# dfm/emcee

Hardware: NVIDIA H100
Metric: walker-steps/sec (nwalkers x iters / s) (higher is better)
Workload: dtype f64

## Files before the change

emcee_b200/csrc/dense_dmma.cu:

```cuda
#include <math.h>

#include "draws.cuh"
#include "engine.cuh"
#include "tma.cuh"

namespace eb {

namespace {

constexpr int DMMA_CONSUMERS = 8;
constexpr int DMMA_THREADS = 64 * DMMA_CONSUMERS;
constexpr int NI = 2;
constexpr int DMMA_PRODUCER_REGS = 64;
constexpr int DMMA_CONSUMER_REGS = 192;
static_assert((DMMA_THREADS / 2) * (DMMA_PRODUCER_REGS + DMMA_CONSUMER_REGS) <= 65536, "register file of one SM");
__host__ __device__ constexpr bool dmma_rebalance(int KB, bool HAS_MEAN, bool BOUNDED) {
  return !BOUNDED && (KB >= 15 || (HAS_MEAN && KB >= 11));
}

__device__ __forceinline__ void dmma1688(double (&c)[4], double2 a01, double2 a23, double b0, double b1) {
  asm volatile(
      "mma.sync.aligned.m16n8k8.row.col.f64.f64.f64.f64 {%0,%1,%2,%3}, {%4,%5,%6,%7}, {%8,%9}, {%0,%1,%2,%3};"
      : "+d"(c[0]), "+d"(c[1]), "+d"(c[2]), "+d"(c[3])
      : "d"(a01.x), "d"(a01.y), "d"(a23.x), "d"(a23.y), "d"(b0), "d"(b1));
}

__host__ __device__ constexpr int col_pairs(int KB) { return (KB + 1) / 2; }
__host__ __device__ constexpr int factor_dmmas(int KB) { return col_pairs(KB) * (KB - col_pairs(KB) + 1); }
__host__ __device__ constexpr size_t factor_doubles(int KB) { return (size_t)factor_dmmas(KB) * 128; }
__host__ __device__ constexpr int row_stride(int KB) { return 8 * KB + 8; }

struct TileMeta {
  double factor[8];
  double log_u[8];
  double lp_old[8];
  int32_t w[8];
};

template <int KB>
struct SmemLayout {
  static constexpr size_t L_doubles = factor_doubles(KB);
  static constexpr size_t mu_doubles = 8 * KB;
  static constexpr size_t slot_doubles = 2 * 8 * row_stride(KB);
  static constexpr size_t off_mu = L_doubles;
  static constexpr size_t off_slots = off_mu + mu_doubles;
  static constexpr size_t off_meta = off_slots + DMMA_CONSUMERS * slot_doubles;
  static constexpr size_t meta_bytes = sizeof(TileMeta) * 2 * DMMA_CONSUMERS;
  static constexpr size_t off_bars_bytes = off_meta * sizeof(double) + meta_bytes;
  static constexpr int nbars = 1 + 3 * DMMA_CONSUMERS;
  static constexpr size_t off_abort_bytes = off_bars_bytes + nbars * sizeof(uint64_t);
  static constexpr size_t off_inbox_bytes = off_abort_bytes + 16;
  static constexpr size_t total_bytes = off_inbox_bytes + sizeof(int32_t) * 2 * 8 * DMMA_CONSUMERS;
};

template <int KB, bool HAS_MEAN>
__device__ __forceinline__ double tile_sumsq(const double (&q)[2 * KB], const double* sL, const double* sMu, int lane,
                                             int g, int t) {
  constexpr int NP = col_pairs(KB);
  double rs0 = 0.0, rs1 = 0.0;
  const double* aptr = sL + 2 * lane;
#pragma unroll
  for (int m0 = 0; m0 < NP; m0 += NI) {
    double c[NI][4];
#pragma unroll
    for (int n = 0; n < NI; ++n) c[n][0] = c[n][1] = c[n][2] = c[n][3] = 0.0;
#pragma unroll
    for (int j = 2 * m0; j < KB; ++j) {
      double x0 = q[2 * j + 0], x1 = q[2 * j + 1];
      if (HAS_MEAN) {
        const double2 m2 = *reinterpret_cast<const double2*>(sMu + 8 * j + 2 * t);
        x0 -= m2.x;
        x1 -= m2.y;
      }
#pragma unroll
      for (int n = 0; n < NI; ++n) {
        if (m0 + n < NP && j >= 2 * (m0 + n)) {
          const double2 a01 = *reinterpret_cast<const double2*>(aptr);
          const double2 a23 = *reinterpret_cast<const double2*>(aptr + 64);
          dmma1688(c[n], a01, a23, x0, x1);
          aptr += 128;
        }
      }
    }
#pragma unroll
    for (int n = 0; n < NI; ++n) {
      rs0 = fma(c[n][0], c[n][0], rs0);
      rs0 = fma(c[n][2], c[n][2], rs0);
      rs1 = fma(c[n][1], c[n][1], rs1);
      rs1 = fma(c[n][3], c[n][3], rs1);
    }
  }
#pragma unroll
  for (int o = 4; o < 32; o <<= 1) {
    rs0 += __shfl_xor_sync(0xffffffffu, rs0, o);
    rs1 += __shfl_xor_sync(0xffffffffu, rs1, o);
  }
  const double e = __shfl_sync(0xffffffffu, rs0, g >> 1), o = __shfl_sync(0xffffffffu, rs1, g >> 1);
  return (g & 1) ? o : e;
}

__device__ __forceinline__ bool grid_wait(const unsigned long long* counter, unsigned long long target, int* status) {
  const long long t0 = clock64();
  while (*reinterpret_cast<const volatile unsigned long long*>(counter) < target) {
    __nanosleep(32);
    if (clock64() - t0 > 60000000000ll) {
      atomicOr(status, FLAG_COMM_TIMEOUT);
      return false;
    }
  }
  __threadfence();
  return true;
}

__device__ __forceinline__ bool peer_wait(const unsigned* my_flags, int rank, int nranks, unsigned target, int lane,
                                          int* status) {
  bool ok = true;
  if (lane < nranks && lane != rank) {
    const volatile unsigned* f = my_flags + lane;
    const long long t0 = clock64();
    while ((int)(*f - target) < 0) {
      __nanosleep(64);
      if (clock64() - t0 > 60000000000ll) {
        atomicOr(status, FLAG_COMM_TIMEOUT);
        ok = false;
        break;
      }
    }
  }
  __threadfence_system();
  return __all_sync(0xffffffffu, ok);
}

template <int KB, bool HAS_MEAN, bool BOUNDED, bool TIMELINE>
__global__ void __launch_bounds__(DMMA_THREADS, 1)
    half_step_dense_dmma_kernel(const HalfStepArgs a, const HalfDesc d0, const HalfDesc* __restrict__ descs,
                                const int nhalf, unsigned long long* gbar, const unsigned long long gbar_base) {
  constexpr int D = 8 * KB;
  constexpr int RS = row_stride(KB);
  using SL = SmemLayout<KB>;
  extern __shared__ __align__(16) unsigned char smem_raw[];
  double* sL = reinterpret_cast<double*>(smem_raw);
  double* sMu = sL + SL::off_mu;
  double* sSlots = sL + SL::off_slots;
  TileMeta* sMeta = reinterpret_cast<TileMeta*>(sL + SL::off_meta);
  uint64_t* bars = reinterpret_cast<uint64_t*>(smem_raw + SL::off_bars_bytes);
  volatile int* sAbort = reinterpret_cast<volatile int*>(smem_raw + SL::off_abort_bytes);
  volatile int* sPeers = sAbort + 1;
  int32_t* sInbox = reinterpret_cast<int32_t*>(smem_raw + SL::off_inbox_bytes);
  uint64_t* barL = bars;
  uint64_t* barFull = bars + 1;
  uint64_t* barReady = bars + 1 + DMMA_CONSUMERS;
  uint64_t* barFree = bars + 1 + 2 * DMMA_CONSUMERS;

  const int tid = threadIdx.x, lane = tid & 31, warp = tid >> 5;
  const bool is_producer = warp >= DMMA_CONSUMERS;
  const int pair = is_producer ? warp - DMMA_CONSUMERS : warp;
  const int g = lane >> 2, t = lane & 3;

  if (tid == 0) {
    *sAbort = 0;
    *sPeers = 0;
    mbar_init(barL, 1);
    for (int c = 0; c < DMMA_CONSUMERS; ++c) {
      mbar_init(barFull + c, 1);
      mbar_init(barReady + c, 1);
      mbar_init(barFree + c, 1);
    }
    asm volatile("fence.mbarrier_init.release.cluster;" ::: "memory");
  }
  if (HAS_MEAN)
    for (int k = tid; k < D; k += DMMA_THREADS) sMu[k] = a.model.params[k];
  __syncthreads();
  const long long t_base = TIMELINE ? clock64() : 0;

  const int tstride = (int)gridDim.x * DMMA_CONSUMERS;
  const int tile0 = (int)blockIdx.x + (int)gridDim.x * pair;
  double* slot = sSlots + (size_t)pair * SL::slot_doubles;
  double* myS = slot + (size_t)g * RS + 2 * t;
  double* myC = myS + 8 * RS;
  TileMeta* meta = sMeta + 2 * pair;
  const bool multi = a.p2p_peer_flags != nullptr;
  unsigned k = 0;

  constexpr bool REBALANCE = dmma_rebalance(KB, HAS_MEAN, BOUNDED);
  if (is_producer) {
    if constexpr (REBALANCE) asm volatile("setmaxnreg.dec.sync.aligned.u32 %0;" ::"n"(DMMA_PRODUCER_REGS));
    long long* tlp = (TIMELINE && lane == 0)
                         ? a.timeline + ((size_t)blockIdx.x * DMMA_CONSUMERS + pair) * TL_TILES * TL_EVENTS : nullptr;
    const double dm1 = (double)a.D - 1.0;
    const int row = lane & 7;
    struct Prep {
      int32_t w, wp;
      double zz, factor, log_u, lp_old;
      bool valid, remote;
    };
    for (int h = 0; h < nhalf; ++h) {
      const HalfDesc d = (h == 0) ? d0 : descs[h];
      const int32_t* order = a.order + (size_t)d.order_step * a.N;
      const int2 rg = a.range ? a.range[(size_t)d.order_step * MAX_SPLITS + d.split] : make_int2(0, d.a_count);
      const int i_lo = rg.x, i_hi = rg.y;
      const int ntiles = (int)(((int64_t)i_hi - i_lo + 7) >> 3);
      const int64_t Nc = a.N - d.a_count;
      const int32_t* aperm = a.aperm ? a.aperm + (size_t)d.order_step * a.N + d.a_start : nullptr;
      auto prep = [&](int tile, bool with_lp) -> Prep {
        Prep p;
        int i = i_lo + tile * 8 + row;
        p.valid = i < i_hi;
        if (!p.valid) i = i_hi - 1;
        if (aperm) i = __ldg(aperm + i);
        const u32x4 A = prop_a(a.seed, d.step, (uint32_t)d.split, (uint32_t)i);
        p.zz = stretch_zz(A, a.p0);
        const int64_t r = stretch_rank(A, Nc);
        p.w = __ldg(order + d.a_start + i);
        p.wp = __ldg(order + complement_slot(r, d.a_start, d.a_count));
        p.log_u = log(accept_uniform(a.seed, d.step, (uint32_t)d.split, (uint32_t)i));
        p.factor = stretch_factor(dm1, p.zz);
        p.lp_old = with_lp ? a.logp[p.w] : 0.0;
        p.remote = multi && (p.wp / a.rows_per_rank != a.p2p_rank);
        return p;
      };
      auto peers_ready = [&]() -> bool {
        if (!multi || *sPeers > h) return true;
        if (pair == 0) {
          if (!peer_wait(a.p2p_my_flags, a.p2p_rank, a.p2p_nranks, a.p2p_wait + (unsigned)h, lane, a.status)) {
            *sAbort = 1;
            return false;
          }
          __syncwarp();
          if (lane == 0) *sPeers = h + 1;
        } else {
          while (*sPeers <= h) {
            if (*sAbort) return false;
            __nanosleep(64);
          }
        }
        asm volatile("fence.proxy.async;" ::: "memory");
        return true;
      };
      auto request = [&](const Prep& p, int lo, int hi) {
        if (lane >= lo && lane < hi) {
          const bool partner = lane >= 8;
          const int32_t wr = partner ? p.wp : p.w;
          const double* base =
              (partner && a.peer_coords != nullptr) ? a.peer_coords[wr / a.rows_per_rank] : a.coords;
          double* dst = slot + (size_t)(partner ? 8 : 0) * RS + (size_t)row * RS;
          if (partner)
            bulk_g2s(dst, base + (size_t)wr * D, (unsigned)(D * sizeof(double)), barFull + pair);
          else
            bulk_g2s_hint(dst, base + (size_t)wr * D, (unsigned)(D * sizeof(double)), barFull + pair,
                          l2_evict_first_policy());
        }
      };
      auto publish = [&](const Prep& p, int par) {
        TileMeta* m = meta + par;
        if (lane < 8) {
          m->factor[row] = p.factor;
          m->log_u[row] = p.log_u;
          m->lp_old[row] = p.lp_old;
          m->w[row] = p.valid ? p.w : -1;
        }
      };
      auto issue = [&](Prep& p, int par, bool load_lp) -> bool {
        if (__any_sync(0xffffffffu, p.remote) && !peers_ready()) return false;
        fence_async_smem();
        if (lane == 0) mbar_arrive_expect_tx(barFull + pair, 16u * D * (unsigned)sizeof(double));
        __syncwarp();
        request(p, 0, 16);
        if (load_lp) p.lp_old = a.logp[p.w];
        publish(p, par);
        return true;
      };
      Prep cur{}, nxt{};
      const bool early = h == 0 && a.dmma_early_own && tile0 < ntiles;
      if (early) {
        cur = prep(tile0, true);
        if (lane == 0) mbar_arrive_expect_tx(barFull + pair, 16u * D * (unsigned)sizeof(double));
        __syncwarp();
        if (tlp) tlp[6] = clock64() - t_base;
        request(cur, 0, 8);
      } else if (tile0 < ntiles) {
        cur = prep(tile0, false);
      }
      if (h == 0) {
        pdl_wait();
        pdl_launch_dependents();
        if (tlp) tlp[10] = clock64() - t_base;
        if (multi && !a.aperm && !peers_ready()) return;
        if (tile0 < ntiles) {
          if (a.dmma_stagger && pair >= DMMA_CONSUMERS / 2)
            mbar_wait_for(barFull + pair - DMMA_CONSUMERS / 2, 0, multi ? 40000 : 12000);
          if (tlp) {
            const long long t_req = clock64() - t_base;
            tlp[11] = t_req;
            if (!early) tlp[6] = t_req;
          }
          if (early) {
            request(cur, 8, 16);
            publish(cur, (int)(k & 1u));
          } else {
            if (!issue(cur, (int)(k & 1u), true)) return;
          }
        }
        if (pair == 0 && !peers_ready()) return;
        if (tile0 + tstride < ntiles) nxt = prep(tile0 + tstride, true);
      } else {
        if (tile0 + tstride < ntiles) nxt = prep(tile0 + tstride, false);
        bool ok = true;
        if (lane == 0) ok = grid_wait(gbar, gbar_base + (unsigned long long)h * gridDim.x, a.status);
        ok = __shfl_sync(0xffffffffu, ok, 0);
        if (!ok) {
          *sAbort = 1;
          return;
        }
        asm volatile("fence.proxy.async;" ::: "memory");
        if (tile0 < ntiles) {
          if (k > 0 && !mbar_wait_abortable(barFree + pair, (k - 1) & 1u, sAbort)) return;
          if (!issue(cur, (int)(k & 1u), true)) return;
        }
      }
      for (int tile = tile0; tile < ntiles; tile += tstride, ++k) {
        const double zz = __shfl_sync(0xffffffffu, cur.zz, g);
        if (!mbar_wait_abortable(barFull + pair, k & 1u, sAbort)) return;
        long long* tlq = (tlp && h == nhalf - 1 && (tile - tile0) / tstride < TL_TILES && lane == 0)
                             ? tlp + ((tile - tile0) / tstride) * TL_EVENTS : nullptr;
        if (tlq) tlq[7] = clock64() - t_base;
        if constexpr (BOUNDED) {
          bool in = true;
#pragma unroll
          for (int j = 0; j < KB; ++j) {
            const double2 s2 = *reinterpret_cast<const double2*>(myS + 8 * j);
            const double2 c2 = *reinterpret_cast<const double2*>(myC + 8 * j);
            const double2 q2 = make_double2(stretch_q(s2.x, c2.x, zz), stretch_q(s2.y, c2.y, zz));
            *reinterpret_cast<double2*>(myC + 8 * j) = q2;
            const double2 l2 = __ldg(reinterpret_cast<const double2*>(a.model.lo + 8 * j + 2 * t));
            const double2 h2 = __ldg(reinterpret_cast<const double2*>(a.model.hi + 8 * j + 2 * t));
            in &= (l2.x <= q2.x) & (q2.x <= h2.x) & (l2.y <= q2.y) & (q2.y <= h2.y);
          }
          in &= __shfl_xor_sync(0xffffffffu, in, 1);
          in &= __shfl_xor_sync(0xffffffffu, in, 2);
          if (t == 0) sInbox[(2 * pair + (k & 1u)) * 8 + g] = in ? 1 : 0;
        } else {
#pragma unroll
          for (int j = 0; j < KB; ++j) {
            const double2 s2 = *reinterpret_cast<const double2*>(myS + 8 * j);
            const double2 c2 = *reinterpret_cast<const double2*>(myC + 8 * j);
            *reinterpret_cast<double2*>(myC + 8 * j) =
                make_double2(stretch_q(s2.x, c2.x, zz), stretch_q(s2.y, c2.y, zz));
          }
        }
        __syncwarp();
        if (lane == 0) mbar_arrive(barReady + pair);
        if (tlq) tlq[8] = clock64() - t_base;
        if (tile + tstride < ntiles) {
          cur = nxt;
          if (!mbar_wait_abortable(barFree + pair, k & 1u, sAbort)) return;
          if (tlq && (tile - tile0) / tstride + 1 < TL_TILES)
            tlq[TL_EVENTS + 6] = clock64() - t_base;
          if (!issue(cur, (int)((k + 1) & 1u), h > 0 && tile == tile0)) return;
          if (tile + 2 * tstride < ntiles) nxt = prep(tile + 2 * tstride, true);
        }
      }
    }
    return;
  }

  if constexpr (REBALANCE) asm volatile("setmaxnreg.inc.sync.aligned.u32 %0;" ::"n"(DMMA_CONSUMER_REGS));
  if (tid == 0) {
    constexpr unsigned bytes = (unsigned)(SL::L_doubles * sizeof(double));
    mbar_arrive_expect_tx(barL, bytes);
    bulk_g2s(sL, a.model.chol, bytes, barL);
  }
  long long* tl = TIMELINE ? a.timeline + ((size_t)blockIdx.x * DMMA_CONSUMERS + pair) * TL_TILES * TL_EVENTS : nullptr;
  pdl_wait();
  pdl_launch_dependents();
  bool alive = mbar_wait_abortable_notrap(barL, 0, sAbort, a.status, FLAG_WAIT_TIMEOUT);
  if (TIMELINE && lane == 0) tl[9] = clock64() - t_base;
  for (int h = 0; h < nhalf; ++h) {
    const HalfDesc d = (h == 0) ? d0 : descs[h];
    const int2 rg = a.range ? a.range[(size_t)d.order_step * MAX_SPLITS + d.split] : make_int2(0, d.a_count);
    const int ntiles = (int)(((int64_t)rg.y - rg.x + 7) >> 3);
    unsigned kk = 0;
    bool peers_passed = false;
    for (int tile = tile0; alive && tile < ntiles; tile += tstride, ++k, ++kk) {
      const TileMeta* m = meta + (k & 1u);
      long long* tlk = (tl && h == nhalf - 1 && kk < TL_TILES && lane == 0) ? tl + kk * TL_EVENTS : nullptr;
      if (tlk) {
        tlk[0] = (long long)tile;
        tlk[1] = clock64() - t_base;
      }
      if (!mbar_wait_abortable_notrap(barReady + pair, k & 1u, sAbort, a.status, FLAG_WAIT_TIMEOUT)) {
        alive = false;
        break;
      }
      if (tlk) tlk[2] = clock64() - t_base;
      double q[2 * KB];
#pragma unroll
      for (int j = 0; j < KB; ++j) {
        const double2 q2 = *reinterpret_cast<const double2*>(myC + 8 * j);
        q[2 * j + 0] = q2.x;
        q[2 * j + 1] = q2.y;
      }
      __syncwarp();
      if (lane == 0) mbar_arrive(barFree + pair);
      if (tlk) tlk[3] = clock64() - t_base;

      const double rs = tile_sumsq<KB, HAS_MEAN>(q, sL, sMu, lane, g, t);
      const int32_t w = m->w[g];
      const double factor = m->factor[g], log_u = m->log_u[g], lp_old = m->lp_old[g];
      const double lp_new = (BOUNDED && sInbox[(2 * pair + (k & 1u)) * 8 + g] == 0) ? -INFINITY : -0.5 * rs;
      if (tlk) tlk[4] = clock64() - t_base;

      if (!isfinite(lp_new)) {
        bool any_inf = false, any_nan = false;
#pragma unroll
        for (int e = 0; e < 2 * KB; ++e) {
          any_inf |= isinf(q[e]);
          any_nan |= isnan(q[e]);
        }
        if (any_inf) atomicOr(a.status, FLAG_INF_PARAM);
        if (any_nan) atomicOr(a.status, FLAG_NAN_PARAM);
        if (isnan(lp_new)) atomicOr(a.status, FLAG_NAN_LOGPROB);
      }

      const double lnpdiff = lnpdiff_red_blue(factor, lp_new, lp_old);
      const bool acc = (w >= 0) && (lnpdiff > log_u);
      if (multi && !peers_passed) {
        while (*sPeers <= h) {
          if (*sAbort) break;
          __nanosleep(64);
        }
        peers_passed = !*sAbort;
        if (!peers_passed) {
          alive = false;
          break;
        }
      }
      if (acc) {
        double* dst = a.coords + (size_t)w * D + 2 * t;
#pragma unroll
        for (int j = 0; j < KB; ++j) *reinterpret_cast<double2*>(dst + 8 * j) = make_double2(q[2 * j], q[2 * j + 1]);
      }
      if (w >= 0 && t == 0) {
        if (acc) {
          a.logp[w] = lp_new;
          atomicAdd(a.nacc + w, 1ull);
        }
        a.accepted[w] = acc ? 1 : 0;
      }
      if (tlk) tlk[5] = clock64() - t_base;
    }
    if (h + 1 < nhalf) {
      __threadfence();
      asm volatile("bar.sync 1, %0;" ::"r"(32 * DMMA_CONSUMERS) : "memory");
      if (*sAbort) alive = false;
      if (tid == 0 && alive) {
        __threadfence();
        atomicAdd(gbar, 1ull);
      }
    }
  }
  if (multi) {
    __threadfence_system();
    asm volatile("bar.sync 1, %0;" ::"r"(32 * DMMA_CONSUMERS) : "memory");
    if (tid == 0 && !*sAbort) {
      const unsigned prev = atomicAdd(a.p2p_done, 1u);
      if (prev == gridDim.x - 1) {
        *a.p2p_done = 0;
        __threadfence_system();
        for (int r = 0; r < a.p2p_nranks; ++r)
          if (r != a.p2p_rank)
            atomicExch_system(a.p2p_peer_flags[r] + a.p2p_rank, a.p2p_signal + (unsigned)(nhalf - 1));
      }
    }
  }
}

template <int KB, bool HAS_MEAN>
__global__ void __launch_bounds__(256) logprob_dense_dmma_kernel(const ModelDev m, const double* __restrict__ x,
                                                                 const int64_t rows, double* __restrict__ out,
                                                                 int* status) {
  constexpr int D = 8 * KB;
  extern __shared__ __align__(16) unsigned char smem_raw[];
  double* sL = reinterpret_cast<double*>(smem_raw);
  double* sMu = sL + factor_doubles(KB);
  uint64_t* barL = reinterpret_cast<uint64_t*>(sMu + D);
  const int tid = threadIdx.x, lane = tid & 31, warp = tid >> 5;
  const int g = lane >> 2, t = lane & 3;
  if (tid == 0) {
    mbar_init(barL, 1);
    asm volatile("fence.mbarrier_init.release.cluster;" ::: "memory");
  }
  if (HAS_MEAN)
    for (int k = tid; k < D; k += blockDim.x) sMu[k] = m.params[k];
  __syncthreads();
  if (tid == 0) {
    constexpr unsigned bytes = (unsigned)(factor_doubles(KB) * sizeof(double));
    mbar_arrive_expect_tx(barL, bytes);
    bulk_g2s(sL, m.chol, bytes, barL);
  }
  const int64_t ntiles = (rows + 7) >> 3;
  bool waited = false;
  for (int64_t tile = (int64_t)blockIdx.x * 8 + warp; tile < ntiles; tile += (int64_t)gridDim.x * 8) {
    int64_t r = tile * 8 + g;
    const bool valid = r < rows;
    if (!valid) r = rows - 1;
    const double* src = x + (size_t)r * D + 2 * t;
    double q[2 * KB];
    bool any_inf = false, any_nan = false, in = true;
#pragma unroll
    for (int j = 0; j < KB; ++j) {
      const double2 v = __ldcg(reinterpret_cast<const double2*>(src + 8 * j));
      q[2 * j + 0] = v.x;
      q[2 * j + 1] = v.y;
      any_inf |= isinf(v.x) | isinf(v.y);
      any_nan |= isnan(v.x) | isnan(v.y);
      if (m.lo != nullptr) {
        const double2 l2 = __ldg(reinterpret_cast<const double2*>(m.lo + 8 * j + 2 * t));
        const double2 h2 = __ldg(reinterpret_cast<const double2*>(m.hi + 8 * j + 2 * t));
        in &= (l2.x <= v.x) & (v.x <= h2.x) & (l2.y <= v.y) & (v.y <= h2.y);
      }
    }
    in &= __shfl_xor_sync(0xffffffffu, in, 1);
    in &= __shfl_xor_sync(0xffffffffu, in, 2);
    if (valid && any_inf) atomicOr(status, FLAG_INF_PARAM);
    if (valid && any_nan) atomicOr(status, FLAG_NAN_PARAM);
    if (!waited) {
      mbar_wait(barL, 0);
      waited = true;
    }
    const double rs = tile_sumsq<KB, HAS_MEAN>(q, sL, sMu, lane, g, t);
    const double lp = in ? -0.5 * rs : -INFINITY;
    if (valid && t == 0) {
      out[r] = lp;
      if (isnan(lp)) atomicOr(status, FLAG_NAN_LOGPROB);
    }
  }
}

template <int KB>
cudaError_t launch_lp_t(const ModelDev& m, const double* x, int64_t rows, double* out, int* status, int sm_count,
                        cudaStream_t st) {
  const size_t smem = (factor_doubles(KB) + 8 * KB) * sizeof(double) + sizeof(uint64_t);
  const bool has_mean = m.s0 != 0.0;
  auto kern = has_mean ? logprob_dense_dmma_kernel<KB, true> : logprob_dense_dmma_kernel<KB, false>;
  if (smem > 48 * 1024) {
    cudaError_t e = cudaFuncSetAttribute(kern, cudaFuncAttributeMaxDynamicSharedMemorySize, (int)smem);
    if (e != cudaSuccess) return e;
  }
  if (rows <= 0) return cudaSuccess;
  const int64_t want = (((rows + 7) >> 3) + 7) / 8;
  const int grid = (int)(want < 2 * sm_count ? want : 2 * sm_count);
  kern<<<grid, 256, smem, st>>>(m, x, rows, out, status);
  return cudaGetLastError();
}

template <int KB>
cudaError_t launch_t(const HalfStepArgs& a, const HalfDesc& d0, const HalfDesc* descs_dev, int nhalf, int max_count,
                     unsigned long long* gbar, unsigned long long gbar_base, int sm_count, bool pdl, int* grid_out,
                     cudaStream_t st) {
  const size_t smem = SmemLayout<KB>::total_bytes;
  const bool has_mean = a.model.s0 != 0.0;
  const bool bounded = a.model.lo != nullptr;
  const bool timeline = a.timeline != nullptr;
  using Kern = decltype(&half_step_dense_dmma_kernel<KB, false, false, false>);
  static const Kern kerns[8] = {
      half_step_dense_dmma_kernel<KB, false, false, false>, half_step_dense_dmma_kernel<KB, true, false, false>,
      half_step_dense_dmma_kernel<KB, false, true, false>,  half_step_dense_dmma_kernel<KB, true, true, false>,
      half_step_dense_dmma_kernel<KB, false, false, true>,  half_step_dense_dmma_kernel<KB, true, false, true>,
      half_step_dense_dmma_kernel<KB, false, true, true>,   half_step_dense_dmma_kernel<KB, true, true, true>};
  const int variant = (has_mean ? 1 : 0) + (bounded ? 2 : 0) + (timeline ? 4 : 0);
  const Kern kern = kerns[variant];
  static bool configured[8][64] = {};
  int dev = 0;
  cudaGetDevice(&dev);
  if (dev < 0 || dev >= 64 || !configured[variant][dev]) {
    cudaError_t e = cudaFuncSetAttribute(kern, cudaFuncAttributeMaxDynamicSharedMemorySize, (int)smem);
    if (e != cudaSuccess) return e;
    if (dev >= 0 && dev < 64) configured[variant][dev] = true;
  }
  *grid_out = 0;
  if (max_count <= 0 || nhalf <= 0) return cudaSuccess;
  const int64_t ntiles = ((int64_t)max_count + 7) / 8;
  const int grid = (int)(ntiles < sm_count ? ntiles : sm_count);
  *grid_out = grid;
  HalfStepArgs args = a;
  HalfDesc first = d0;
  if (nhalf == 1) {
    cudaLaunchConfig_t cfg{};
    cfg.gridDim = dim3(grid);
    cfg.blockDim = dim3(DMMA_THREADS);
    cfg.dynamicSmemBytes = smem;
    cfg.stream = st;
    cudaLaunchAttribute attr[1];
    attr[0].id = cudaLaunchAttributeProgrammaticStreamSerialization;
    attr[0].val.programmaticStreamSerializationAllowed = 1;
    cfg.attrs = attr;
    cfg.numAttrs = pdl ? 1 : 0;
    return cudaLaunchKernelEx(&cfg, kern, args, first, descs_dev, nhalf, gbar, gbar_base);
  }
  void* params[] = {(void*)&args, (void*)&first, (void*)&descs_dev, (void*)&nhalf, (void*)&gbar, (void*)&gbar_base};
  return cudaLaunchCooperativeKernel((const void*)kern, dim3(grid), dim3(DMMA_THREADS), params, smem, st);
}

}

bool dense_dmma_supported(int D) { return D >= 8 && D <= 128 && D % 8 == 0; }

size_t dense_dmma_factor_doubles(int D) { return factor_doubles(D / 8); }

void dense_dmma_pack_factor(const double* L, int D, double* packed) {
  const int KB = D / 8, NP = col_pairs(KB);
  size_t idx = 0;
  for (int m0 = 0; m0 < NP; m0 += NI)
    for (int j = 2 * m0; j < KB; ++j)
      for (int n = 0; n < NI; ++n) {
        const int m = m0 + n;
        if (m >= NP || j < 2 * m) continue;
        for (int half = 0; half < 2; ++half)
          for (int lane = 0; lane < 32; ++lane) {
            const int g = lane >> 2, t = lane & 3, row = 8 * j + 2 * t + half;
            for (int hi = 0; hi < 2; ++hi) {
              const int col = 16 * m + 8 * hi + g;
              packed[idx++] = (col < D && col <= row) ? L[(size_t)row * D + col] : 0.0;
            }
          }
      }
}

cudaError_t launch_logprob_dense_dmma(const ModelDev& m, int D, const double* x, int64_t rows, double* out,
                                      int* status, int sm_count, cudaStream_t st) {
#define EB_LP_CASE(KB) \
  case 8 * KB:         \
    return launch_lp_t<KB>(m, x, rows, out, status, sm_count, st);
  switch (D) {
    EB_LP_CASE(1)
    EB_LP_CASE(2)
    EB_LP_CASE(3)
    EB_LP_CASE(4)
    EB_LP_CASE(5)
    EB_LP_CASE(6)
    EB_LP_CASE(7)
    EB_LP_CASE(8)
    EB_LP_CASE(9)
    EB_LP_CASE(10)
    EB_LP_CASE(11)
    EB_LP_CASE(12)
    EB_LP_CASE(13)
    EB_LP_CASE(14)
    EB_LP_CASE(15)
    EB_LP_CASE(16)
  }
#undef EB_LP_CASE
  return cudaErrorNotSupported;
}

cudaError_t launch_dense_dmma(const HalfStepArgs& a, const HalfDesc& d0, const HalfDesc* descs_dev, int nhalf,
                              int max_count, unsigned long long* gbar, unsigned long long gbar_base, int sm_count,
                              bool pdl, int* grid_out, cudaStream_t st) {
#define EB_DMMA_CASE(KB) \
  case 8 * KB:           \
    return launch_t<KB>(a, d0, descs_dev, nhalf, max_count, gbar, gbar_base, sm_count, pdl, grid_out, st);
  switch (a.D) {
    EB_DMMA_CASE(1)
    EB_DMMA_CASE(2)
    EB_DMMA_CASE(3)
    EB_DMMA_CASE(4)
    EB_DMMA_CASE(5)
    EB_DMMA_CASE(6)
    EB_DMMA_CASE(7)
    EB_DMMA_CASE(8)
    EB_DMMA_CASE(9)
    EB_DMMA_CASE(10)
    EB_DMMA_CASE(11)
    EB_DMMA_CASE(12)
    EB_DMMA_CASE(13)
    EB_DMMA_CASE(14)
    EB_DMMA_CASE(15)
    EB_DMMA_CASE(16)
  }
#undef EB_DMMA_CASE
  return cudaErrorNotSupported;
}

}
```

Before: 995.2 million.

## Move stretch-move computation from producer warp into consumers reading TMA data directly

The producer warp no longer waits for the bulk copy to land and then computes the stretched proposal back into shared memory. Consumers now wait on the TMA full barrier, compute q from the complementary and own coordinates with zz published in the tile metadata, and do the bounds check themselves. A separate per-parity ready barrier signals when the metadata is published. This removes a shared-memory round trip and a producer-consumer handoff from the critical path, at the cost of more consumer work and an extra barrier wait.

Result: no change. 988.1 million (median of 6 runs) (-0.7%).

```diff
diff --git a/emcee_b200/csrc/dense_dmma.cu b/emcee_b200/csrc/dense_dmma.cu
--- a/emcee_b200/csrc/dense_dmma.cu
+++ b/emcee_b200/csrc/dense_dmma.cu
@@ -31,6 +31,7 @@
 __host__ __device__ constexpr int row_stride(int KB) { return 8 * KB + 8; }
 
 struct TileMeta {
+  double zz[8];
   double factor[8];
   double log_u[8];
   double lp_old[8];
@@ -47,10 +48,9 @@
   static constexpr size_t off_meta = off_slots + DMMA_CONSUMERS * slot_doubles;
   static constexpr size_t meta_bytes = sizeof(TileMeta) * 2 * DMMA_CONSUMERS;
   static constexpr size_t off_bars_bytes = off_meta * sizeof(double) + meta_bytes;
-  static constexpr int nbars = 1 + 3 * DMMA_CONSUMERS;
+  static constexpr int nbars = 1 + 4 * DMMA_CONSUMERS;
   static constexpr size_t off_abort_bytes = off_bars_bytes + nbars * sizeof(uint64_t);
-  static constexpr size_t off_inbox_bytes = off_abort_bytes + 16;
-  static constexpr size_t total_bytes = off_inbox_bytes + sizeof(int32_t) * 2 * 8 * DMMA_CONSUMERS;
+  static constexpr size_t total_bytes = off_abort_bytes + 16;
 };
 
 template <int KB, bool HAS_MEAN>
@@ -146,11 +146,10 @@
   uint64_t* bars = reinterpret_cast<uint64_t*>(smem_raw + SL::off_bars_bytes);
   volatile int* sAbort = reinterpret_cast<volatile int*>(smem_raw + SL::off_abort_bytes);
   volatile int* sPeers = sAbort + 1;
-  int32_t* sInbox = reinterpret_cast<int32_t*>(smem_raw + SL::off_inbox_bytes);
   uint64_t* barL = bars;
   uint64_t* barFull = bars + 1;
-  uint64_t* barReady = bars + 1 + DMMA_CONSUMERS;
-  uint64_t* barFree = bars + 1 + 2 * DMMA_CONSUMERS;
+  uint64_t* barFree = bars + 1 + DMMA_CONSUMERS;
+  uint64_t* barReady = bars + 1 + 2 * DMMA_CONSUMERS;
 
   const int tid = threadIdx.x, lane = tid & 31, warp = tid >> 5;
   const bool is_producer = warp >= DMMA_CONSUMERS;
@@ -163,8 +162,9 @@
     mbar_init(barL, 1);
     for (int c = 0; c < DMMA_CONSUMERS; ++c) {
       mbar_init(barFull + c, 1);
-      mbar_init(barReady + c, 1);
       mbar_init(barFree + c, 1);
+      mbar_init(barReady + 2 * c, 1);
+      mbar_init(barReady + 2 * c + 1, 1);
     }
     asm volatile("fence.mbarrier_init.release.cluster;" ::: "memory");
   }
@@ -176,8 +176,8 @@
   const int tstride = (int)gridDim.x * DMMA_CONSUMERS;
   const int tile0 = (int)blockIdx.x + (int)gridDim.x * pair;
   double* slot = sSlots + (size_t)pair * SL::slot_doubles;
-  double* myS = slot + (size_t)g * RS + 2 * t;
-  double* myC = myS + 8 * RS;
+  const double* myS = slot + (size_t)g * RS + 2 * t;
+  const double* myC = myS + 8 * RS;
   TileMeta* meta = sMeta + 2 * pair;
   const bool multi = a.p2p_peer_flags != nullptr;
   unsigned k = 0;
@@ -187,6 +187,9 @@
     if constexpr (REBALANCE) asm volatile("setmaxnreg.dec.sync.aligned.u32 %0;" ::"n"(DMMA_PRODUCER_REGS));
     long long* tlp = (TIMELINE && lane == 0)
                          ? a.timeline + ((size_t)blockIdx.x * DMMA_CONSUMERS + pair) * TL_TILES * TL_EVENTS : nullptr;
+    auto stamp = [&](int i, int ev) {
+      if (tlp && i < TL_TILES) tlp[i * TL_EVENTS + ev] = clock64() - t_base;
+    };
     const double dm1 = (double)a.D - 1.0;
     const int row = lane & 7;
     struct Prep {
@@ -251,6 +254,12 @@
                           l2_evict_first_policy());
         }
       };
+      auto arm = [&](const Prep& p, int par) {
+        if (lane < 8) meta[par].zz[row] = p.zz;
+        __syncwarp();
+        if (lane == 0) mbar_arrive_expect_tx(barFull + pair, 16u * D * (unsigned)sizeof(double));
+        __syncwarp();
+      };
       auto publish = [&](const Prep& p, int par) {
         TileMeta* m = meta + par;
         if (lane < 8) {
@@ -259,12 +268,12 @@
           m->lp_old[row] = p.lp_old;
           m->w[row] = p.valid ? p.w : -1;
         }
+        __syncwarp();
+        if (lane == 0) mbar_arrive(barReady + 2 * pair + par);
       };
       auto issue = [&](Prep& p, int par, bool load_lp) -> bool {
         if (__any_sync(0xffffffffu, p.remote) && !peers_ready()) return false;
-        fence_async_smem();
-        if (lane == 0) mbar_arrive_expect_tx(barFull + pair, 16u * D * (unsigned)sizeof(double));
-        __syncwarp();
+        arm(p, par);
         request(p, 0, 16);
         if (load_lp) p.lp_old = a.logp[p.w];
         publish(p, par);
@@ -274,8 +283,7 @@
       const bool early = h == 0 && a.dmma_early_own && tile0 < ntiles;
       if (early) {
         cur = prep(tile0, true);
-        if (lane == 0) mbar_arrive_expect_tx(barFull + pair, 16u * D * (unsigned)sizeof(double));
-        __syncwarp();
+        arm(cur, (int)(k & 1u));
         if (tlp) tlp[6] = clock64() - t_base;
         request(cur, 0, 8);
       } else if (tile0 < ntiles) {
@@ -300,6 +308,7 @@
           } else {
             if (!issue(cur, (int)(k & 1u), true)) return;
           }
+          if (h == nhalf - 1) stamp(0, 8);
         }
         if (pair == 0 && !peers_ready()) return;
         if (tile0 + tstride < ntiles) nxt = prep(tile0 + tstride, true);
@@ -315,48 +324,19 @@
         asm volatile("fence.proxy.async;" ::: "memory");
         if (tile0 < ntiles) {
           if (k > 0 && !mbar_wait_abortable(barFree + pair, (k - 1) & 1u, sAbort)) return;
+          if (h == nhalf - 1) stamp(0, 6);
           if (!issue(cur, (int)(k & 1u), true)) return;
+          if (h == nhalf - 1) stamp(0, 8);
         }
       }
       for (int tile = tile0; tile < ntiles; tile += tstride, ++k) {
-        const double zz = __shfl_sync(0xffffffffu, cur.zz, g);
-        if (!mbar_wait_abortable(barFull + pair, k & 1u, sAbort)) return;
-        long long* tlq = (tlp && h == nhalf - 1 && (tile - tile0) / tstride < TL_TILES && lane == 0)
-                             ? tlp + ((tile - tile0) / tstride) * TL_EVENTS : nullptr;
-        if (tlq) tlq[7] = clock64() - t_base;
-        if constexpr (BOUNDED) {
-          bool in = true;
-#pragma unroll
-          for (int j = 0; j < KB; ++j) {
-            const double2 s2 = *reinterpret_cast<const double2*>(myS + 8 * j);
-            const double2 c2 = *reinterpret_cast<const double2*>(myC + 8 * j);
-            const double2 q2 = make_double2(stretch_q(s2.x, c2.x, zz), stretch_q(s2.y, c2.y, zz));
-            *reinterpret_cast<double2*>(myC + 8 * j) = q2;
-            const double2 l2 = __ldg(reinterpret_cast<const double2*>(a.model.lo + 8 * j + 2 * t));
-            const double2 h2 = __ldg(reinterpret_cast<const double2*>(a.model.hi + 8 * j + 2 * t));
-            in &= (l2.x <= q2.x) & (q2.x <= h2.x) & (l2.y <= q2.y) & (q2.y <= h2.y);
-          }
-          in &= __shfl_xor_sync(0xffffffffu, in, 1);
-          in &= __shfl_xor_sync(0xffffffffu, in, 2);
-          if (t == 0) sInbox[(2 * pair + (k & 1u)) * 8 + g] = in ? 1 : 0;
-        } else {
-#pragma unroll
-          for (int j = 0; j < KB; ++j) {
-            const double2 s2 = *reinterpret_cast<const double2*>(myS + 8 * j);
-            const double2 c2 = *reinterpret_cast<const double2*>(myC + 8 * j);
-            *reinterpret_cast<double2*>(myC + 8 * j) =
-                make_double2(stretch_q(s2.x, c2.x, zz), stretch_q(s2.y, c2.y, zz));
-          }
-        }
-        __syncwarp();
-        if (lane == 0) mbar_arrive(barReady + pair);
-        if (tlq) tlq[8] = clock64() - t_base;
         if (tile + tstride < ntiles) {
+          const int i = (tile - tile0) / tstride + 1;
           cur = nxt;
           if (!mbar_wait_abortable(barFree + pair, k & 1u, sAbort)) return;
-          if (tlq && (tile - tile0) / tstride + 1 < TL_TILES)
-            tlq[TL_EVENTS + 6] = clock64() - t_base;
+          if (h == nhalf - 1) stamp(i, 6);
           if (!issue(cur, (int)((k + 1) & 1u), h > 0 && tile == tile0)) return;
+          if (h == nhalf - 1) stamp(i, 8);
           if (tile + 2 * tstride < ntiles) nxt = prep(tile + 2 * tstride, true);
         }
       }
@@ -388,26 +368,47 @@
         tlk[0] = (long long)tile;
         tlk[1] = clock64() - t_base;
       }
-      if (!mbar_wait_abortable_notrap(barReady + pair, k & 1u, sAbort, a.status, FLAG_WAIT_TIMEOUT)) {
+      if (!mbar_wait_abortable_notrap(barFull + pair, k & 1u, sAbort, a.status, FLAG_WAIT_TIMEOUT)) {
         alive = false;
         break;
       }
       if (tlk) tlk[2] = clock64() - t_base;
       double q[2 * KB];
-#pragma unroll
-      for (int j = 0; j < KB; ++j) {
-        const double2 q2 = *reinterpret_cast<const double2*>(myC + 8 * j);
-        q[2 * j + 0] = q2.x;
-        q[2 * j + 1] = q2.y;
+      {
+        const double zz = m->zz[g];
+#pragma unroll
+        for (int j = 0; j < KB; ++j) {
+          const double2 s2 = *reinterpret_cast<const double2*>(myS + 8 * j);
+          const double2 c2 = *reinterpret_cast<const double2*>(myC + 8 * j);
+          q[2 * j + 0] = stretch_q(s2.x, c2.x, zz);
+          q[2 * j + 1] = stretch_q(s2.y, c2.y, zz);
+        }
       }
       __syncwarp();
       if (lane == 0) mbar_arrive(barFree + pair);
       if (tlk) tlk[3] = clock64() - t_base;
 
       const double rs = tile_sumsq<KB, HAS_MEAN>(q, sL, sMu, lane, g, t);
+      while (!mbar_try_wait(barReady + 2 * pair + (k & 1u), (k >> 1) & 1u))
+        if (*sAbort) break;
+      if (*sAbort) {
+        alive = false;
+        break;
+      }
+      bool in = true;
+      if constexpr (BOUNDED) {
+#pragma unroll
+        for (int j = 0; j < KB; ++j) {
+          const double2 l2 = __ldg(reinterpret_cast<const double2*>(a.model.lo + 8 * j + 2 * t));
+          const double2 h2 = __ldg(reinterpret_cast<const double2*>(a.model.hi + 8 * j + 2 * t));
+          in &= (l2.x <= q[2 * j]) & (q[2 * j] <= h2.x) & (l2.y <= q[2 * j + 1]) & (q[2 * j + 1] <= h2.y);
+        }
+        in &= __shfl_xor_sync(0xffffffffu, in, 1);
+        in &= __shfl_xor_sync(0xffffffffu, in, 2);
+      }
       const int32_t w = m->w[g];
       const double factor = m->factor[g], log_u = m->log_u[g], lp_old = m->lp_old[g];
-      const double lp_new = (BOUNDED && sInbox[(2 * pair + (k & 1u)) * 8 + g] == 0) ? -INFINITY : -0.5 * rs;
+      const double lp_new = in ? -0.5 * rs : -INFINITY;
       if (tlk) tlk[4] = clock64() - t_base;
 
       if (!isfinite(lp_new)) {
```
